# marianaGarcez/SpatialFlink

Measured on AMD Instinct MI355X. Metric: points/sec per window (kNN k=50, range r) at 1/2/4/8 MI355X; % HBM roofline, higher is better.
Workload: dtype f64

## Files before the change

### spatialflink_amd/csrc/gf_internal.hpp

```cpp
#pragma once

#include <hip/hip_runtime.h>

#include <cstdint>
#include <string>
#include <vector>

#include "../../include/geoflink_hip.h"
#include "gf_text.hpp"
#include "gf_numerics.hpp"

struct gf_ctx {
  int device = 0;
  hipStream_t stream = nullptr;
  hipStream_t own_stream = nullptr;
  std::string last_error;
  int timing = 0;
  int timing_period = 1;
  int64_t timing_seq[GF_K_COUNT] = {};
  struct Ev { hipEvent_t a, b; int kid; };
  std::vector<Ev> pending;
  std::vector<hipEvent_t> pool;
  std::vector<hipEvent_t> order_pool;
  double acc_ms[GF_K_COUNT] = {};
  int64_t acc_n[GF_K_COUNT] = {};
  void* scratch = nullptr;
  size_t scratch_bytes = 0;
  void* pinned = nullptr;
  size_t pinned_bytes = 0;
  int num_cus = 256;
  int join_legacy = 0;
  int join_coarse = 0;
  int join_stream = 0;
  int geojson_walk = 0;
  int geojson_wave = 0;
  unsigned long long* geojson_check = nullptr;
  int64_t csv_mean_line[2] = {0, 0};
  int join_async_done = 0;
  double join_ppp = 0.0;
  hipStream_t aux = nullptr;
  hipStream_t aux2 = nullptr;
  gf_objid_dict* dict = nullptr;
  unsigned long long* expand_ticket = nullptr;
  unsigned long long expand_base = 0;
  unsigned long long* expand_status = nullptr;
  int64_t expand_status_cap = 0;
  uint32_t expand_epoch = 0;
  unsigned long long* join_gctr = nullptr;
  unsigned long long* join_hint = nullptr;
  void* csv_head = nullptr;
  uint64_t* join_hist = nullptr;
  unsigned long long* join_ovf = nullptr;
  int64_t join_hint_no = 0;
};

struct gf_objid_dict {
  gf_ctx* ctx = nullptr;
  void* slots = nullptr;
  uint64_t cap = 0;
  char* arena = nullptr;
  uint64_t arena_cap = 0;
  unsigned long long* counters = nullptr;
  unsigned long long* idmap = nullptr;
  uint64_t idmap_cap = 0;
  int64_t size = 0;
  uint32_t round = 2;
  void* work[3] = {nullptr, nullptr, nullptr};
  uint64_t work_cap = 0;
  uint32_t* slot_of = nullptr;
  uint32_t* flag = nullptr;
  uint32_t* rank = nullptr;
  uint32_t* tmp = nullptr;
  uint64_t line_cap = 0;
  char* src = nullptr;
  uint64_t src_cap = 0;
  std::vector<unsigned long long> h_idmap;
  std::vector<char> h_arena;
};

namespace gf {

int set_err(gf_ctx* ctx, int code, const std::string& msg);
int hip_err(gf_ctx* ctx, hipError_t e, const char* what);
void* ctx_scratch(gf_ctx* ctx, size_t bytes, int* status);
int sync_aux(gf_ctx* ctx);
void* ctx_pinned(gf_ctx* ctx, size_t bytes, int* status);
int bind(gf_ctx* ctx);

#define GF_HIP_CHECK(ctx, call)                                   \
  do {                                                            \
    hipError_t _e = (call);                                       \
    if (_e != hipSuccess) return ::gf::hip_err((ctx), _e, #call); \
  } while (0)
// ... 36 lines not shown
struct KnnState {
  uint32_t hist[kDistBins];
  uint32_t ticket;
  uint32_t pad;
  double T;
  double s_pre;
  unsigned long long count;
  double hint_T;
  unsigned long long tr[4];
  unsigned long long maybe;
};

struct KnnScanArgs {
  const double* x;
  const double* y;
  const int64_t* objID;
  int64_t begin, end;
  double qx, qy;
  QueryRect qr;
  double T, s_pre;
  int use_state;
  int metric;
  KnnState* st;
  double* cand_d;
  uint32_t* cand_i;
  int64_t* cand_o;
  unsigned long long cap;
};

struct KnnSampleArgs {
  const double* x;
  const double* y;
  int64_t n;
  double qx, qy;
  QueryRect qr;
  double r, s_r;
  int32_t k;
  int metric;
  int use_hint;
  KnnState* st;
};

struct PolyView {
  const int32_t* ring_off;
  const int32_t* vert_off;
  const double* vx;
  const double* vy;
  const double* ring_env;
  int metric;
  const uint8_t* rect;
};

constexpr int kChainRun = 32;
constexpr int kChainPlainRuns = 2;
constexpr int kChainPlainRunsValue = 4;
struct ChainView {
  const int32_t* run_off;
  const int32_t* vert_off;
  const double* vx;
  const double* vy;
  const double* run_env;
  int metric;
};

struct KnnPolyArgs {
  const double* x;
  const double* y;
  const int64_t* objID;
  int64_t begin, end;
  QueryRect qr;
  PolyView poly;
  double bbox[4];
  int approx;
  double r;
  int32_t k;
  int use_state;
  int use_hint;
  KnnState* st;
  double* cand_d;
  uint32_t* cand_i;
  int64_t* cand_o;
  unsigned long long cap;
  uint32_t* maybe_i;
};

struct KnnSelectArgs {
  KnnState* st;
  const double* cand_d;
  const uint32_t* cand_i;
  const int64_t* cand_o;
  unsigned long long cap;
  int use_state;
  double T;
  double r;
  int32_t k;
  int write_hint;
  int64_t idx_base;
  void* result;
};

constexpr int kRangeMaxParts = 4096;
constexpr int kRangeTicketSlot = 2 * kRangeMaxParts;

struct RangeArgs {
  const double* x;
  const double* y;
  int64_t n;
  uint64_t* bitmap;
  uint64_t* multi;
  uint64_t* partials;
  int64_t* counts;
  int32_t nq;
  QueryRect qr;
  int32_t grid_n;
  double minX, minY, cl;
  const uint8_t* table;
  const uint32_t* rows;
  const uint32_t* rowoff;
  const uint8_t* spans;
  int32_t span_bytes;
  int32_t span_lds;
  const double* xt;
  const double* yt;
  double x_lo, x_hi, y_lo, y_hi;
  double sx_lo, sx_hi;
  double sy_lo, sy_hi;
  int span_mode;
  double inv_cl;
  const int32_t* extra;
  int32_t n_extra;
  const int32_t* cand_off;
  const int32_t* cand_list;
  int approx;
  int metric;
  double r, s_r;
  double thr;
  double qx0, qy0;
  const double* qx;
  const double* qy;
  int32_t npoly;
  const int32_t* ring_off;
  const int32_t* vert_off;
  const double* vx;
  const double* vy;
  const double* bbox;
  const double* ring_env;
  uint32_t* queue;
  uint32_t* queue_count;
  double* queue_xy;
  int64_t seg_cap;
  int32_t drain_lanes;
  const uint8_t* rect;
  const int32_t* brect;
  int32_t g_layers, c_layers;
};

hipError_t launch_assign(gf_ctx* ctx, const gf_grid* g, const gf_points* p, int32_t* cx, int32_t* cy);
hipError_t launch_histogram(hipStream_t s, const uint32_t* keys, int64_t n, uint32_t* hist);
constexpr int kRadixMaxBits = 9;
constexpr int kRadixMaxDigits = 1 << kRadixMaxBits;
constexpr int kRadixThreads = 1024;
constexpr int kRadixTile = 8192;
#ifndef GF_BUCKET_BITS
#define GF_BUCKET_BITS 9
#endif
constexpr int kBucketBits = GF_BUCKET_BITS;
// ... 447 lines not shown
  int64_t nt;
  uint32_t* tlist[2];
  uint32_t* tlen[2];
  const uint32_t* toff[2];
  int64_t m, npts;
  int64_t* c_keys;
  double* c_x;
  double* c_y;
  int64_t* c_ts;
  uint32_t* c_idx;
};
enum TjoinStage {
  kTjoinQueryKeys = 0,
  kTjoinQueryRank = 1,
  kTjoinQueryScatter = 2,
  kTjoinRunStarts = 3,
  kTjoinRunEnds = 4,
  kTjoinCellKeys = 5,
  kTjoinProbe = 6,
  kTjoinOccupied = 7,
  kTjoinCompact = 8,
  kTjoinRows = 9,
  kTjoinRowSlots = 10,
  kTjoinSideList = 11,
  kTjoinTotals = 12,
  kTjoinGather = 13,
};
hipError_t launch_tjoin(gf_ctx* ctx, int stage, const TjoinArgs& a);

struct TrangeArgs {
  const double* x;
  const double* y;
  int64_t n;
  const uint32_t* did;
  uint32_t* hit;
  uint64_t* bitmap;
  int32_t grid_n;
  double minX, minY, cl;
  const uint8_t* cls;
  const int32_t* cand_off;
  const int32_t* cand_list;
  const int32_t* extra;
  int32_t n_extra;
  PolyView poly;
  const uint8_t* wide;
  uint2* work;
  uint32_t work_cap;
  unsigned long long* ctr;
  int64_t* count;
};
enum TrangeStage {
  kTrangeMark = 0,
  kTrangeWaves = 1,
  kTrangeCount = 2,
};
hipError_t launch_trange(gf_ctx* ctx, int stage, const TrangeArgs& a);

hipError_t launch_knn_sample(gf_ctx* ctx, const KnnSampleArgs& a);
hipError_t launch_knn_scan(gf_ctx* ctx, const KnnScanArgs& a, int blocks, int unroll, int nt);
hipError_t launch_knn_select(gf_ctx* ctx, const KnnSelectArgs& a);
struct KnnLargeArgs {
  const double* cd;
  const int64_t* co;
  const uint32_t* ci;
  uint32_t* perm;
  int64_t m;
  int field;
  uint32_t* keys;
  uint32_t* out;
  uint32_t* cnt;
  int pass;
  unsigned long long* lane_count;
  unsigned long long* lane_maybe;
  int32_t k;
  double T;
  int64_t idx_base;
  void* result;
};
hipError_t launch_knn_large(gf_ctx* ctx, int op, const KnnLargeArgs& a);
constexpr int32_t kMaxKLarge = 1 << 24;
int knn_exact_record(gf_knn_plan* P, const gf_points* pts, void* result);

hipError_t launch_knn_poly_sample(gf_ctx* ctx, const KnnPolyArgs& a, int chain);
hipError_t launch_knn_poly_scan(gf_ctx* ctx, const KnnPolyArgs& a, int blocks, int chain);
struct KnnSelectArgs;
struct KnnMergeArgs;
hipError_t launch_knn_poly_fused(gf_ctx* ctx, const KnnPolyArgs& a, const KnnSelectArgs& prev, int has_prev,
                                 int blocks, const KnnMergeArgs* merge, int chain);
__host__ __device__ inline size_t merge_any_hash(int64_t e) {
  size_t h = 1024;
  while (h < 2 * (size_t)e) h <<= 1;
  return h;
}
__host__ __device__ inline size_t merge_any_bytes(int32_t nrec, int32_t k) {
  const int64_t e = (int64_t)nrec * k;
  return ((size_t)e * 24 + merge_any_hash(e) * 12 + 255) & ~(size_t)255;
}
hipError_t launch_knn_merge(gf_ctx* ctx, int32_t k, const void* records, int32_t nrec, size_t rec_stride,
                            int32_t nwin, size_t win_stride, void* result, size_t res_stride, int foreign,
                            void* scratch);
__host__ __device__ inline size_t str_side_off(int32_t k) { return ((size_t)4 * (k + 1) + 7) & ~(size_t)7; }
__host__ __device__ inline size_t str_record_bytes(int32_t k, int64_t cap) {
  return 32 + (size_t)24 * k + 16 + str_side_off(k) + (((size_t)cap + 7) & ~(size_t)7);
}
__host__ __device__ inline size_t strmerge_pow2(int64_t e) {
  size_t p = 2;
  while (p < (size_t)e) p <<= 1;
  return p;
}
__host__ __device__ inline size_t strmerge_bytes(int32_t nrec, int32_t k) {
  const int64_t e = (int64_t)nrec * k;
  return ((size_t)e * 40 + strmerge_pow2(e) * 4 + strmerge_pow2(2 * e) * 8 + (size_t)k * 16 + 1024) & ~(size_t)255;
}
hipError_t launch_knn_attach_strings(gf_ctx* ctx, int32_t k, const unsigned long long* idmap, const char* arena,
                                     int64_t dict_size, const void* records, int32_t nrec, int64_t cap, void* out);
hipError_t launch_knn_merge_strings(gf_ctx* ctx, int32_t k, int64_t cap, const void* records, int32_t nrec,
                                    size_t rec_stride, int32_t nwin, size_t win_stride, void* results, void* scratch);
constexpr int kMaxMergeRecs = 64;
struct KnnRecList {
  const char* rec[kMaxMergeRecs];
};
hipError_t launch_knn_merge_list(gf_ctx* ctx, int32_t k, const KnnRecList& list, int32_t nrec, void* result,
                                 void* scratch);
constexpr int kFusedMergeMaxK = 128;
struct KnnMergeArgs {
  int32_t nrec;
  void* result;
  KnnRecList list;
};
hipError_t launch_knn_fused(gf_ctx* ctx, const KnnScanArgs& a, const KnnSelectArgs& prev, int has_prev,
                            int scan_blocks, int unroll, int nt, const KnnMergeArgs* merge);
int knn_enqueue_merge(gf_knn_plan* P, const gf_points* pts, void* result, const KnnMergeArgs* merge, int* merged);
bool knn_select_pending(const gf_knn_plan* P);

hipError_t launch_range(gf_ctx* ctx, const RangeArgs& a, int table_mode, int poly, int blocks);
struct RangeWin {
  const double* x;
  const double* y;
  int64_t n;
  uint64_t* bitmap;
  uint64_t* multi;
  uint64_t* partials;
  int64_t* counts;
};
struct RangeBatch {
  RangeWin w[kRangeBatchMax];
};
hipError_t launch_range_batch(gf_ctx* ctx, const RangeArgs& a, const RangeBatch& b, int nwin, int table_mode, int poly,
                              int blocks);
struct RangeGatherArgs {
  const uint32_t* list[kMaxMergeRecs];
  const int64_t* cnt[kMaxMergeRecs];
  int64_t base[kMaxMergeRecs];
  int32_t npanes;
  int64_t total;
  uint32_t* out;
  int64_t* count;
};
hipError_t launch_range_window_gather(hipStream_t s, const RangeGatherArgs& a);
hipError_t launch_join_ppoly(gf_ctx* ctx, const RangeArgs& a, int blocks, int jblocks, uint32_t* ecnt, uint32_t* ecand,
                             uint32_t* btot, unsigned long long* total, uint32_t* pairs, int64_t cap, int aligned,
                             int poly);

struct JoinArgs {
  const double* ox;
  const double* oy;
  int64_t no;
  double u_minX, u_minY, u_cl;
  int32_t qn;
  int64_t c;
  const uint32_t* q_off;
// ... 143 lines not shown
  int64_t span_bytes = 0;
  double* xt = nullptr;
  double* yt = nullptr;
  double x_lo = 0, x_hi = 0, y_lo = 0, y_hi = 0;
  double sx_lo = 0, sx_hi = 0;
  double sy_lo = 0, sy_hi = 0;
  double span_frac = 1.0;
  int32_t* extra = nullptr;
  int32_t n_extra = 0;
  int32_t* cand_off = nullptr;
  int32_t* cand_list = nullptr;
  double* qx = nullptr;
  double* qy = nullptr;
  int32_t npoly = 0;
  int32_t* ring_off = nullptr;
  int32_t* vert_off = nullptr;
  double* vx = nullptr;
  double* vy = nullptr;
  double* bbox = nullptr;
  double* ring_env = nullptr;
  uint64_t* partials = nullptr;
  uint64_t* batch_partials = nullptr;
  int blocks = 0;
  uint32_t* queue = nullptr;
  double* queue_xy = nullptr;
  int64_t queue_cap = 0;
  uint32_t* queue_count = nullptr;
  int64_t cls_cells[4] = {0, 0, 0, 0};
  int32_t scan_blocks = 0;
  int32_t defer_mode = 0;
  int32_t drain_lanes = 0;
  int join = 0;
  int32_t* brect = nullptr;
  uint8_t* rect = nullptr;
  uint32_t* jecnt = nullptr;
  uint32_t* jecand = nullptr;
  uint32_t* jbtot = nullptr;
  unsigned long long* jtotal = nullptr;
  int chain_mode = 0;
  int32_t* run_off = nullptr;
  double* run_env = nullptr;
};

struct gf_knn_plan {
  gf_ctx* ctx = nullptr;
  gf_grid grid{};
  double qx = 0, qy = 0, r = 0;
  int32_t k = 0;
  int metric = 0;
  gf::QueryRect qr{};
  struct Lane {
    gf::KnnState* st = nullptr;
    double* cand_d = nullptr;
    uint32_t* cand_i = nullptr;
    int64_t* cand_o = nullptr;
  } lane[6];
  int64_t cap = 0;
  int pipeline = 1;
  uint64_t seq = 0;
  int lane_warm[6] = {0, 0, 0, 0, 0, 0};
  struct Pend {
    int lane;
    void* result;
    int64_t idx_base;
    uint64_t seq;
  };
  Pend pq[3];
  int npq = 0;
  int use_hint = 1;
  int64_t idx_base = 0;
  void* tmp_result = nullptr;
  void* host_result = nullptr;
  int scan_blocks = 0;
  int scan_unroll = 2;
  int scan_nt = 1;
  int large = 0;
  int poly = 0, approx = 0;
  int32_t* ring_off = nullptr;
  int32_t* vert_off = nullptr;
  double* vx = nullptr;
  double* vy = nullptr;
  double* ring_env = nullptr;
  double bbox[4] = {0, 0, 0, 0};
  uint32_t* maybe_i[3] = {nullptr, nullptr, nullptr};
  int64_t maybe_cap = 0;
  int chain_mode = 0;
};

struct gf_window {
  gf_ctx* ctx = nullptr;
  int64_t capacity = 0, n = 0;
  double* x = nullptr;
  double* y = nullptr;
  int64_t* objID = nullptr;
  int64_t* ts = nullptr;
  bool has_objid = false, has_ts = false;
  const int64_t* objid_mapped = nullptr;
  hipStream_t copy = nullptr;
  hipEvent_t ready = nullptr, fence_main = nullptr, fence_aux = nullptr, fence_aux2 = nullptr;
  bool pending = false;
};
```

### spatialflink_amd/csrc/k_knn.hip

```cpp
#define GF_TU_NAME k_knn_hip
#include "gf_buildtag.hpp"

#include <type_traits>

#include "gf_geom.hpp"
#include "gf_internal.hpp"

namespace gf {

__device__ __forceinline__ bool classify_cg(const QueryRect& q, double px, double py) {
  const double xs = (px == px) ? px : q.minX;
  const double ys = (py == py) ? py : q.minY;
  const bool inG = q.g_any && in_iv(q.gx, xs) && in_iv(q.gy, ys);
  return inG || (in_iv(q.cgx, xs) && in_iv(q.cgy, ys));
}

template <int METRIC>
__device__ __forceinline__ bool knn_pass(double qx, double qy, const QueryRect& qr, double px, double py,
                                         double sp, double T) {
  const double dx = qx - px, dy = qy - py;
  const double s = dx * dx + dy * dy;
  if (!(s <= sp)) return false;
  if (!classify_cg(qr, px, py)) return false;
  return METRIC == 0 ? true : fdlibm_hypot(dx, dy) <= T;
// ... 1072 lines not shown
                                                               void* result) {
  __shared__ SelFull L;
  const ListRecs src{&list};
  knn_merge_body(k, src, nrec, result, L);
}

hipError_t launch_knn_merge(gf_ctx* ctx, int32_t k, const void* records, int32_t nrec, size_t rec_stride,
                            int32_t nwin, size_t win_stride, void* result, size_t res_stride, int foreign,
                            void* scratch) {
  KTimer t(ctx, GF_K_KNN_MERGE);
  if (k > kMaxK)
    hipLaunchKernelGGL(knn_merge_any_kernel, dim3(nwin), dim3(kMergeAnyT), 0, ctx->stream, k, (const char*)records,
                       nrec, rec_stride, win_stride, result, res_stride, foreign, (char*)scratch,
                       merge_any_bytes(nrec, k));
  else
    hipLaunchKernelGGL(knn_merge_kernel, dim3(nwin), dim3(kSelT), 0, ctx->stream, k, (const char*)records, nrec,
                       rec_stride, win_stride, result, res_stride, foreign);
  return hipGetLastError();
}

hipError_t launch_knn_merge_list(gf_ctx* ctx, int32_t k, const KnnRecList& list, int32_t nrec, void* result,
                                 void* scratch) {
  KTimer t(ctx, GF_K_KNN_MERGE);
  if (k > kMaxK)
    hipLaunchKernelGGL(knn_merge_any_list_kernel, dim3(1), dim3(kMergeAnyT), 0, ctx->stream, k, list, nrec, result,
                       (char*)scratch);
  else
    hipLaunchKernelGGL(knn_merge_list_kernel, dim3(1), dim3(kSelT), 0, ctx->stream, k, list, nrec, result);
  return hipGetLastError();
}

template <int CHAIN>
__device__ __forceinline__ double poly_exact_distance(const KnnPolyArgs& a, double px, double py, double T) {
  if constexpr (CHAIN)
    return chain_distance<true>(px, py, ChainView{a.poly.ring_off, a.poly.vert_off, a.poly.vx, a.poly.vy, a.poly.ring_env,
                                                  a.poly.metric}, 0, T);
  else
    return polygon_distance(px, py, a.poly, 0);
}

template <int CHAIN>
__device__ __forceinline__ bool poly_pass(const KnnPolyArgs& a, double px, double py, double T, double& d) {
  if (!classify_cg(a.qr, px, py)) return false;
  if (px == px && py == py && env_far(a.bbox, px, py, T)) return false;
  d = a.approx ? point_bbox_distance(px, py, a.bbox) : poly_exact_distance<CHAIN>(a, px, py, T);
  return d <= T;
}

template <int CHAIN>
__global__ __launch_bounds__(kBlock) void knn_poly_sample_kernel(KnnPolyArgs a) {
  __shared__ uint32_t lh[kDistBins];
  if (a.use_hint) {
    const double h = a.st->hint_T;
    if (h > 0.0) {
      if (blockIdx.x == 0 && threadIdx.x == 0) a.st->T = h < a.r ? h : a.r;
      return;
    }
  }
  for (int j = threadIdx.x; j < kDistBins; j += kBlock) lh[j] = 0u;
  __syncthreads();
  const int64_t n = a.end - a.begin;
  const int64_t stride = n / gridDim.x;
  const int64_t p0 = a.begin + (int64_t)blockIdx.x * stride;
  const int64_t bbase = dist_bin_base(a.r);
  for (int u = threadIdx.x; u < kSamplePerBlock; u += kBlock) {
    const double px = a.x[p0 + u], py = a.y[p0 + u];
    double d;
    if (poly_pass<CHAIN>(a, px, py, a.r, d)) atomicAdd(&lh[dist_bin(d, bbase)], 1u);
  }
  sample_finish(a.st, lh, a.k, a.r, a.poly.metric, bbase);
}

__device__ __forceinline__ bool poly_maybe(const KnnPolyArgs& a, double px, double py, double T) {
  if (!classify_cg(a.qr, px, py)) return false;
  return !(px == px && py == py && env_far(a.bbox, px, py, T));
}

__device__ __forceinline__ void maybe_append(const KnnPolyArgs& a, bool c, int64_t i) {
  wave_reserve(&a.st->maybe, c, [&](unsigned long long pos) {
    if (pos < a.cap) a.maybe_i[pos] = (uint32_t)i;
  });
}

__device__ __forceinline__ void knn_poly_scan_body(const KnnPolyArgs& a, double T, int64_t bid, int64_t nblk) {
  const int lane = threadIdx.x & 63;
  const int64_t stride = nblk * kBlock;
  const int64_t pb = a.begin >> 1, pe = a.end >> 1;
  for (int64_t p = pb + bid * kBlock + threadIdx.x; p - lane < pe; p += stride) {
    const bool in = p < pe;
    dbl2 xv = {0.0, 0.0}, yv = {0.0, 0.0};
    if (in) {
      xv = __builtin_nontemporal_load(reinterpret_cast<const dbl2*>(a.x) + p);
      yv = __builtin_nontemporal_load(reinterpret_cast<const dbl2*>(a.y) + p);
    }
    const bool c0 = in && poly_maybe(a, xv.x, yv.x, T);
    const bool c1 = in && poly_maybe(a, xv.y, yv.y, T);
    if (__ballot(c0 || c1) == 0) continue;
    maybe_append(a, c0, 2 * p);
    maybe_append(a, c1, 2 * p + 1);
  }
  if ((a.end & 1) && bid == 0 && threadIdx.x < 64) {
    const int64_t i = a.end - 1;
    maybe_append(a, lane == 0 && poly_maybe(a, a.x[i], a.y[i], T), i);
  }
}

__global__ __launch_bounds__(kBlock) void knn_poly_scan_kernel(KnnPolyArgs a) {
  knn_poly_scan_body(a, a.use_state ? a.st->T : a.r, blockIdx.x, gridDim.x);
}

__global__ __launch_bounds__(kBlock) void knn_poly_fused_kernel(KnnPolyArgs a, KnnSelectArgs prev, int has_prev,
                                                                KnnMergeArgs m) {
  __shared__ SelLite L;
  if (blockIdx.x == 0) {
    fused_block0(prev, has_prev, m, L);
    return;
  }
  double T;
  if (a.use_state == 2) {
    T = a.st->T;
  } else {
    const double h = a.st->hint_T;
    T = (h > 0.0 && h < a.r) ? h : a.r;
    if (blockIdx.x == 1 && threadIdx.x == 0) a.st->T = T;
  }
  knn_poly_scan_body(a, T, blockIdx.x - 1, gridDim.x - 1);
}

template <int CHAIN>
__global__ __launch_bounds__(kBlock) void knn_poly_refine_kernel(KnnPolyArgs a) {
  const double T = a.use_state ? a.st->T : a.r;
  const unsigned long long nm = a.st->maybe;
  if (nm > a.cap) {
    if (blockIdx.x == 0 && threadIdx.x == 0) atomicAdd(&a.st->count, nm);
    return;
  }
  const int lane = threadIdx.x & 63;
  const int64_t stride = (int64_t)gridDim.x * kBlock;
  for (int64_t j = (int64_t)blockIdx.x * kBlock + threadIdx.x; j - lane < (int64_t)nm; j += stride) {
    const bool in = j < (int64_t)nm;
    const int64_t i = in ? (int64_t)a.maybe_i[j] : 0;
    double d = 0.0;
    bool c = false;
    if (in) {
      const double px = a.x[i], py = a.y[i];
      d = a.approx ? point_bbox_distance(px, py, a.bbox) : poly_exact_distance<CHAIN>(a, px, py, T);
      c = d <= T;
    }
    wave_reserve(&a.st->count, c, [&a, d, i](unsigned long long pos) {
      if (pos < a.cap) {
        a.cand_d[pos] = d;
        a.cand_i[pos] = (uint32_t)i;
        a.cand_o[pos] = a.objID[i];
      }
    });
  }
}

hipError_t launch_knn_poly_sample(gf_ctx* ctx, const KnnPolyArgs& a, int chain) {
  KTimer t(ctx, GF_K_KNN_SAMPLE);
  if (chain) hipLaunchKernelGGL(knn_poly_sample_kernel<1>, dim3(kSampleBlocks), dim3(kBlock), 0, ctx->stream, a);
  else hipLaunchKernelGGL(knn_poly_sample_kernel<0>, dim3(kSampleBlocks), dim3(kBlock), 0, ctx->stream, a);
  return hipGetLastError();
}

static void launch_knn_poly_refine(gf_ctx* ctx, const KnnPolyArgs& a, int chain) {
  if (chain) hipLaunchKernelGGL(knn_poly_refine_kernel<1>, dim3(256), dim3(kBlock), 0, ctx->stream, a);
  else hipLaunchKernelGGL(knn_poly_refine_kernel<0>, dim3(256), dim3(kBlock), 0, ctx->stream, a);
}

hipError_t launch_knn_poly_fused(gf_ctx* ctx, const KnnPolyArgs& a, const KnnSelectArgs& prev, int has_prev,
                                 int blocks, const KnnMergeArgs* merge, int chain) {
  KnnMergeArgs m{};
  if (merge && has_prev) m = *merge;
  {
    KTimer t(ctx, GF_K_KNN_SCAN);
    hipLaunchKernelGGL(knn_poly_fused_kernel, dim3(blocks + 1), dim3(kBlock), 0, ctx->stream, a, prev, has_prev, m);
  }
  KnnPolyArgs r = a;
  r.use_state = 1;
  launch_knn_poly_refine(ctx, r, chain);
  return hipGetLastError();
}

hipError_t launch_knn_poly_scan(gf_ctx* ctx, const KnnPolyArgs& a, int blocks, int chain) {
  {
    KTimer t(ctx, GF_K_KNN_SCAN);
    hipLaunchKernelGGL(knn_poly_scan_kernel, dim3(blocks), dim3(kBlock), 0, ctx->stream, a);
  }
  launch_knn_poly_refine(ctx, a, chain);
  return hipGetLastError();
}

struct StrSide {
  int32_t status;
  int32_t n;
  int64_t nbytes;
};
__device__ __forceinline__ StrSide* side_of(void* rec, int32_t k) {
  return reinterpret_cast<StrSide*>((char*)rec + 32 + (size_t)24 * k);
}
__device__ __forceinline__ uint32_t* side_off(void* rec, int32_t k) { return reinterpret_cast<uint32_t*>(side_of(rec, k) + 1); }
__device__ __forceinline__ char* side_bytes(void* rec, int32_t k) { return (char*)side_off(rec, k) + str_side_off(k); }
__device__ __forceinline__ bool dict_key(int64_t o) { return o < GF_OBJID_NUMERIC_MIN; }

template <int NT>
__device__ __forceinline__ uint32_t block_excl(uint32_t v, uint32_t* excl, uint32_t* ws) {
  const int lane = threadIdx.x & 63, w = threadIdx.x >> 6;
  uint32_t inc = v;
#pragma unroll
  for (int o = 1; o < 64; o <<= 1) {
    const uint32_t t = __shfl_up(inc, o, 64);
    if (lane >= o) inc += t;
  }
  if (lane == 63) ws[w] = inc;
  __syncthreads();
  uint32_t before = 0, tot = 0;
#pragma unroll
  for (int i = 0; i < NT / 64; ++i) {
    before += i < w ? ws[i] : 0u;
    tot += ws[i];
  }
  *excl = before + inc - v;
  __syncthreads();
  return tot;
}

template <int NT, class Len, class Src>
__device__ void side_pack(void* rec, int32_t k, int n, int64_t cap, const Len& len_of, const Src& src_of, uint32_t* ws) {
  StrSide* sd = side_of(rec, k);
  uint32_t* off = side_off(rec, k);
  char* bytes = side_bytes(rec, k);
  uint32_t carry = 0;
  for (int i0 = 0; i0 < n; i0 += NT) {
    const int i = i0 + (int)threadIdx.x;
    const uint32_t l = i < n ? len_of(i) : 0u;
    uint32_t ex;
    const uint32_t tot = block_excl<NT>(l, &ex, ws);
    if (i < n) off[i] = carry + ex;
    carry += tot;
  }
  const bool fits = (int64_t)carry <= cap;
  if (fits)
    for (int i = threadIdx.x; i < n; i += NT) {
      const uint32_t l = len_of(i);
      const char* src = src_of(i);
      char* dst = bytes + off[i];
      for (uint32_t b = 0; b < l; ++b) dst[b] = src[b];
    }
  if (threadIdx.x == 0) {
    off[n] = carry;
    sd->status = fits ? 0 : 1;
    sd->n = n;
    sd->nbytes = (int64_t)carry;
  }
}

__global__ __launch_bounds__(kBlock) void knn_attach_strings_kernel(int32_t k, const unsigned long long* idmap,
                                                                    const char* arena, int64_t dict_size,
                                                                    const char* records, int64_t cap, char* out) {
  __shared__ uint32_t ws[kBlock / 64];
  const size_t rb = 32 + (size_t)24 * k;
  const char* in = records + (size_t)blockIdx.x * rb;
  char* o = out + (size_t)blockIdx.x * str_record_bytes(k, cap);
  for (size_t b = (size_t)threadIdx.x * 8; b < rb; b += (size_t)kBlock * 8)
    *reinterpret_cast<uint64_t*>(o + b) = *reinterpret_cast<const uint64_t*>(in + b);
  const gf_knn_header* h = reinterpret_cast<const gf_knn_header*>(in);
  const int n = h->status == 0 ? h->n : 0;
  const RecView v = rec_view((void*)in, k);
  auto meta = [&](int i) -> unsigned long long {
    const int64_t key = v.o[i];
// ... 182 lines not shown
```

### spatialflink_amd/csrc/knn.cpp

```cpp
#define GF_TU_NAME knn_cpp
#include "gf_buildtag.hpp"

#include <hip/hip_runtime.h>

#include <initializer_list>
#include <iterator>
#include <limits>
#include <unordered_set>

#include "gf_chain_plan.hpp"
#include "gf_host.hpp"

using namespace gf;

extern "C" size_t gf_knn_result_bytes(int32_t k) {
  return sizeof(gf_knn_header) + (size_t)(k > 0 ? k : 0) * (sizeof(double) + 2 * sizeof(int64_t));
}

extern "C" void gf_knn_plan_destroy(gf_knn_plan* P) {
  if (!P) return;
  hipSetDevice(P->ctx->device);
  hipStreamSynchronize(P->ctx->stream);
  for (auto& L : P->lane) {
    if (L.st) hipFree(L.st);
// ... 11 lines not shown
}

static int knn_alloc_lane(gf_knn_plan* P, int j, int64_t cap) {
  gf_ctx* ctx = P->ctx;
  gf_knn_plan::Lane& L = P->lane[j];
  if (!L.st) {
    GF_HIP_CHECK(ctx, hipMalloc(&L.st, sizeof(KnnState)));
    GF_HIP_CHECK(ctx, hipMemset(L.st, 0, sizeof(KnnState)));
  }
  if (L.cand_d) hipFree(L.cand_d);
  if (L.cand_i) hipFree(L.cand_i);
  if (L.cand_o) hipFree(L.cand_o);
  L.cand_d = nullptr;
  L.cand_i = nullptr;
  L.cand_o = nullptr;
  GF_HIP_CHECK(ctx, hipMalloc(&L.cand_d, sizeof(double) * (size_t)cap));
  GF_HIP_CHECK(ctx, hipMalloc(&L.cand_i, sizeof(uint32_t) * (size_t)cap));
  GF_HIP_CHECK(ctx, hipMalloc(&L.cand_o, sizeof(int64_t) * (size_t)cap));
  return GF_OK;
}

static int knn_alloc_candidates(gf_knn_plan* P, int64_t cap) {
  int st;
  GF_HIP_CHECK(P->ctx, hipStreamSynchronize(P->ctx->stream));
  if (int e = sync_aux(P->ctx)) return e;
  for (int j = 0; j < (int)std::size(P->lane); ++j)
    if ((j == 0 || P->lane[j].st) && (st = knn_alloc_lane(P, j, cap))) return st;
  P->cap = cap;
  return GF_OK;
}

extern "C" int gf_knn_pp_plan_create(gf_ctx* ctx, const gf_grid* g, double qx, double qy, double r, int32_t k,
                                     int metric, gf_knn_plan** out) {
  if (!ctx || !out || !grid_ok(g) || k < 1 || k > kMaxKLarge || (metric != 0 && metric != 1))
    return set_err(ctx, GF_ERR_ARG, "gf_knn_pp_plan_create: bad argument (k must be in [1, 2^24])");
  *out = nullptr;
  int st = bind(ctx);
  if (st) return st;
  gf_knn_plan* P = new gf_knn_plan();
  P->ctx = ctx;
  P->grid = *g;
  P->qx = qx; P->qy = qy; P->r = r; P->k = k; P->metric = metric;
  const int32_t gl = guaranteed_layers(g->cellLength, r), cl = candidate_layers(g->cellLength, r);
  const int32_t qcx = cell_index(qx, g->minX, g->cellLength), qcy = cell_index(qy, g->minY, g->cellLength);
  P->qr = make_qrect(*g, qcx, qcy, gl, cl);
  auto fail = [&](int s) { gf_knn_plan_destroy(P); return s; };
  hipError_t e;
  if ((st = knn_alloc_candidates(P, (int64_t)1 << 20))) return fail(st);
  if ((e = hipMalloc(&P->tmp_result, gf_knn_result_bytes(k))) != hipSuccess) return fail(hip_err(ctx, e, "hipMalloc"));
  if ((e = hipHostMalloc(&P->host_result, gf_knn_result_bytes(k), hipHostMallocDefault)) != hipSuccess)
    return fail(hip_err(ctx, e, "hipHostMalloc"));
  P->scan_blocks = 0;
  P->large = k > kMaxK;
  *out = P;
  return GF_OK;
}

static void bbox_query_rect(gf_knn_plan* P, const gf_grid* g, double r) {
  const int32_t gl = guaranteed_layers(g->cellLength, r), cl = candidate_layers(g->cellLength, r);
  const int64_t bx0 = cell_index(P->bbox[0], g->minX, g->cellLength), bx1 = cell_index(P->bbox[2], g->minX, g->cellLength);
  const int64_t by0 = cell_index(P->bbox[1], g->minY, g->cellLength), by1 = cell_index(P->bbox[3], g->minY, g->cellLength);
  const double nan = std::numeric_limits<double>::quiet_NaN();
  const int64_t n1 = g->n - 1;
  QueryRect q;
  q.minX = g->minX;
  q.minY = g->minY;
  if (cl > 0) {
    q.cgx = axis_iv(std::max<int64_t>(bx0 - cl, 0), std::min<int64_t>(bx1 + cl, n1), g->minX, g->cellLength);
    q.cgy = axis_iv(std::max<int64_t>(by0 - cl, 0), std::min<int64_t>(by1 + cl, n1), g->minY, g->cellLength);
  } else {
    q.cgx = q.cgy = {nan, nan};
  }
  if (gl > 0) {
    q.gx = axis_iv(std::max<int64_t>(bx0 - gl, 0), std::min<int64_t>(bx1 + gl, n1), g->minX, g->cellLength);
    q.gy = axis_iv(std::max<int64_t>(by0 - gl, 0), std::min<int64_t>(by1 + gl, n1), g->minY, g->cellLength);
  } else if (gl == 0) {
    q.gx = axis_iv(bx0, bx1, g->minX, g->cellLength);
    q.gy = axis_iv(by0, by1, g->minY, g->cellLength);
  } else {
    q.gx = q.gy = {nan, nan};
  }
  q.g_any = (gl >= 0) && !std::isnan(q.gx.lo) && !std::isnan(q.gy.lo);
  P->qr = q;
}

extern "C" int gf_knn_ppoly_plan_create(gf_ctx* ctx, const gf_grid* g, const gf_polygons* poly, double r,
                                        int32_t k, int approximate, int metric, gf_knn_plan** out) {
  if (!ctx || !out || !grid_ok(g) || !poly || poly->npoly != 1 || k < 1 || k > kMaxKLarge || (metric != 0 && metric != 1))
    return set_err(ctx, GF_ERR_ARG, "gf_knn_ppoly_plan_create: bad argument (one polygon, 1 <= k <= 2^24)");
  *out = nullptr;
  const int32_t nrings = poly->ring_off[1] - poly->ring_off[0];
  if (poly->ring_off[0] != 0 || nrings < 1) return set_err(ctx, GF_ERR_ARG, "polygon without a shell");
  for (int32_t j = 0; j < nrings; ++j) {
    const int32_t v0 = poly->vert_off[j], v1 = poly->vert_off[j + 1];
    if (v1 - v0 < 4 || poly->vx[v0] != poly->vx[v1 - 1] || poly->vy[v0] != poly->vy[v1 - 1])
      return set_err(ctx, GF_ERR_ARG, "ring must be closed with >= 4 vertices");
  }
  int st = gf_knn_pp_plan_create(ctx, g, 0.0, 0.0, r, k, metric, out);
  if (st) return st;
  gf_knn_plan* P = *out;
  *out = nullptr;
  P->poly = 1;
  P->approx = approximate != 0;
  std::vector<double> renv(4 * (size_t)nrings);
  for (int32_t j = 0; j < nrings; ++j) {
    const int32_t v0 = poly->vert_off[j], v1 = poly->vert_off[j + 1];
    double mnx = poly->vx[v0], mxx = mnx, mny = poly->vy[v0], mxy = mny;
    for (int32_t v = v0 + 1; v < v1; ++v) {
      mnx = std::min(mnx, poly->vx[v]); mxx = std::max(mxx, poly->vx[v]);
      mny = std::min(mny, poly->vy[v]); mxy = std::max(mxy, poly->vy[v]);
    }
    renv[4 * j] = mnx; renv[4 * j + 1] = mxx; renv[4 * j + 2] = mny; renv[4 * j + 3] = mxy;
  }
  P->bbox[0] = renv[0]; P->bbox[1] = renv[2]; P->bbox[2] = renv[1]; P->bbox[3] = renv[3];
  bbox_query_rect(P, g, r);
  const int32_t nverts = poly->vert_off[nrings];
  std::vector<int32_t> ro = {0, nrings}, vo(poly->vert_off, poly->vert_off + nrings + 1);
  std::vector<double> vx(poly->vx, poly->vx + nverts), vy(poly->vy, poly->vy + nverts);
  if ((st = upload(ctx, &P->ring_off, ro)) || (st = upload(ctx, &P->vert_off, vo)) || (st = upload(ctx, &P->vx, vx)) ||
      (st = upload(ctx, &P->vy, vy)) || (st = upload(ctx, &P->ring_env, renv))) {
    gf_knn_plan_destroy(P);
    return st;
  }
  *out = P;
  return GF_OK;
}

extern "C" int gf_knn_pls_plan_create(gf_ctx* ctx, const gf_grid* g, const gf_linestrings* lines, double r,
                                      int32_t k, int approximate, int metric, gf_knn_plan** out) {
  if (!ctx || !out || !grid_ok(g) || !chain_valid(lines) || lines->nline != 1 || k < 1 || k > kMaxKLarge ||
      (metric != 0 && metric != 1))
    return set_err(ctx, GF_ERR_ARG, "gf_knn_pls_plan_create: bad argument (one line of >= 2 vertices, 1 <= k <= 2^24)");
  *out = nullptr;
  int st = gf_knn_pp_plan_create(ctx, g, 0.0, 0.0, r, k, metric, out);
  if (st) return st;
  gf_knn_plan* P = *out;
  *out = nullptr;
  P->poly = 2;
  P->approx = approximate != 0;
  ChainTables T;
  chain_build(*lines, kChainRun, T);
  for (int i = 0; i < 4; ++i) P->bbox[i] = T.bbox[i];
  bbox_query_rect(P, g, r);
  if ((st = upload(ctx, &P->ring_off, T.run_off)) || (st = upload(ctx, &P->vert_off, T.vert_off)) ||
      (st = upload(ctx, &P->vx, T.vx)) || (st = upload(ctx, &P->vy, T.vy)) || (st = upload(ctx, &P->ring_env, T.run_env))) {
    gf_knn_plan_destroy(P);
    return st;
  }
  *out = P;
  return GF_OK;
}

extern "C" int gf_knn_plan_set_chain_mode(gf_knn_plan* P, int mode) {
  if (!P || P->poly != 2 || (mode != 0 && mode != 1)) return GF_ERR_ARG;
  P->chain_mode = mode;
  return GF_OK;
}

extern "C" int gf_knn_plan_set_capacity(gf_knn_plan* P, int64_t cap) {
  if (!P || cap < 2 || cap > (int64_t)1 << 31) return GF_ERR_ARG;
  int st = bind(P->ctx);
  if (st) return st;
  int fs = gf_knn_plan_flush(P);
  if (fs) return fs;
  hipStreamSynchronize(P->ctx->stream);
  return knn_alloc_candidates(P, cap & ~(int64_t)1);
}

extern "C" int gf_knn_plan_set_tuning(gf_knn_plan* P, int32_t scan_blocks, int32_t unroll, int32_t nontemporal) {
  if (!P || scan_blocks < 0 || unroll < 1 || unroll > 8) return GF_ERR_ARG;
  P->scan_blocks = scan_blocks;
  P->scan_unroll = unroll;
  P->scan_nt = nontemporal != 0;
  return GF_OK;
}

extern "C" int gf_knn_plan_set_index_base(gf_knn_plan* P, int64_t base) {
  if (!P || base < 0) return GF_ERR_ARG;
  P->idx_base = base;
  return GF_OK;
}

static int knn_streams(const gf_knn_plan* P) { return P->pipeline >= 2 ? P->pipeline - 1 : 1; }

static hipStream_t knn_stream(gf_ctx* ctx, int s) { return s == 0 ? ctx->stream : (s == 1 ? ctx->aux : ctx->aux2); }

static KnnScanArgs scan_args(gf_knn_plan* P, int j, const gf_points* pts, int64_t begin, int64_t end, int use_state) {
  const gf_knn_plan::Lane& L = P->lane[j];
  KnnScanArgs s{};
  s.x = pts->x; s.y = pts->y; s.objID = pts->objID; s.begin = begin; s.end = end;
  s.qx = P->qx; s.qy = P->qy; s.qr = P->qr;
  s.T = P->r; s.s_pre = s_prefilter(P->r, P->metric);
  s.use_state = use_state; s.metric = P->metric; s.st = L.st;
  s.cand_d = L.cand_d; s.cand_i = L.cand_i; s.cand_o = L.cand_o; s.cap = (unsigned long long)P->cap;
  return s;
}

static KnnSelectArgs select_args(gf_knn_plan* P, int j, int use_state, int write_hint, void* result,
                                 int64_t idx_base) {
  const gf_knn_plan::Lane& L = P->lane[j];
  KnnSelectArgs q{};
  q.st = L.st; q.cand_d = L.cand_d; q.cand_i = L.cand_i; q.cand_o = L.cand_o;
  q.cap = (unsigned long long)P->cap;
  q.use_state = use_state; q.T = P->r; q.r = P->r; q.k = P->k; q.result = result;
  q.write_hint = write_hint; q.idx_base = idx_base;
  return q;
}

static KnnPolyArgs poly_args(gf_knn_plan* P, int j, const gf_points* pts, int64_t begin, int64_t end, int use_state,
                             int use_hint) {
  const gf_knn_plan::Lane& L = P->lane[j];
  KnnPolyArgs a{};
  a.x = pts->x; a.y = pts->y; a.objID = pts->objID; a.begin = begin; a.end = end;
  a.qr = P->qr;
  a.poly = PolyView{P->ring_off, P->vert_off, P->vx, P->vy, P->ring_env, P->metric};
  if (P->poly == 2 && P->chain_mode == 1) a.poly.ring_off = nullptr;
  for (int i = 0; i < 4; ++i) a.bbox[i] = P->bbox[i];
  a.approx = P->approx; a.r = P->r; a.k = P->k; a.use_state = use_state; a.use_hint = use_hint;
  a.st = L.st; a.cand_d = L.cand_d; a.cand_i = L.cand_i; a.cand_o = L.cand_o; a.cap = (unsigned long long)P->cap;
  a.maybe_i = P->maybe_i[j % knn_streams(P)];
  return a;
}

static int poly_buffers(gf_knn_plan* P) {
  if (P->maybe_cap >= P->cap) return GF_OK;
  GF_HIP_CHECK(P->ctx, hipStreamSynchronize(P->ctx->stream));
  if (int e = sync_aux(P->ctx)) return e;
  for (auto& m : P->maybe_i) {
    if (m) hipFree(m);
    m = nullptr;
    GF_HIP_CHECK(P->ctx, hipMalloc(&m, sizeof(uint32_t) * (size_t)P->cap));
  }
  P->maybe_cap = P->cap;
  return GF_OK;
}

static int scan_blocks_for(gf_knn_plan* P, int64_t n) {
  if (P->scan_blocks > 0) return P->scan_blocks;
  const int64_t pairs = ((P->poly ? (n + 1) / 2 : n) + 1) / 2;
  return std::min(stream_blocks(P->ctx, pairs), P->ctx->num_cus * 4);
}

static int launch_sample(gf_knn_plan* P, int j, const gf_points* pts, int use_hint) {
  if (P->poly) {
    GF_HIP_CHECK(P->ctx, launch_knn_poly_sample(P->ctx, poly_args(P, j, pts, 0, pts->n, 1, use_hint), P->poly == 2));
    return GF_OK;
  }
  KnnSampleArgs s{};
  s.x = pts->x; s.y = pts->y; s.n = pts->n; s.qx = P->qx; s.qy = P->qy; s.qr = P->qr;
  s.r = P->r; s.s_r = s_prefilter(P->r, P->metric); s.k = P->k; s.metric = P->metric; s.st = P->lane[j].st;
  s.use_hint = use_hint;
  GF_HIP_CHECK(P->ctx, launch_knn_sample(P->ctx, s));
  return GF_OK;
}

static int launch_scan(gf_knn_plan* P, int j, const gf_points* pts, int64_t begin, int64_t end, int use_state) {
  gf_ctx* ctx = P->ctx;
  const int blocks = scan_blocks_for(P, end - begin);
  if (P->poly) {
    if (int st = poly_buffers(P)) return st;
    GF_HIP_CHECK(ctx, launch_knn_poly_scan(ctx, poly_args(P, j, pts, begin, end, use_state, 0), blocks, P->poly == 2));
  } else {
    GF_HIP_CHECK(ctx, launch_knn_scan(ctx, scan_args(P, j, pts, begin, end, use_state), blocks, P->scan_unroll,
                                      P->scan_nt));
  }
  return GF_OK;
}

static int launch_fused(gf_knn_plan* P, int j, const gf_points* pts, int use_state, const KnnSelectArgs& prev,
                        int has_prev, const KnnMergeArgs* merge) {
  gf_ctx* ctx = P->ctx;
  const int blocks = scan_blocks_for(P, pts->n);
  if (P->poly) {
    if (int st = poly_buffers(P)) return st;
    GF_HIP_CHECK(ctx, launch_knn_poly_fused(ctx, poly_args(P, j, pts, 0, pts->n, use_state, 0), prev, has_prev, blocks,
                                           merge, P->poly == 2));
  } else {
    GF_HIP_CHECK(ctx, launch_knn_fused(ctx, scan_args(P, j, pts, 0, pts->n, use_state), prev, has_prev, blocks,
                                       P->scan_unroll, P->scan_nt, merge));
  }
  return GF_OK;
}

static bool fallback_resamples(const gf_knn_plan* P) { return !P->poly; }

static int knn_scan_select(gf_knn_plan* P, int j, const gf_points* pts, int64_t begin, int64_t end, int use_state,
                           int write_hint, void* result) {
  if (int st = launch_scan(P, j, pts, begin, end, use_state)) return st;
  GF_HIP_CHECK(P->ctx, launch_knn_select(P->ctx, select_args(P, j, use_state, write_hint, result, P->idx_base)));
  return GF_OK;
}

static int knn_large(gf_knn_plan* P, const gf_points* pts, void* result) {
  gf_ctx* ctx = P->ctx;
  int st;
  const int64_t n = pts->n;
  if (P->cap < n && (st = knn_alloc_candidates(P, n))) return st;
  if ((st = launch_scan(P, 0, pts, 0, n, 0))) return st;
  const gf_knn_plan::Lane& L = P->lane[0];
  const int64_t mm = std::max<int64_t>(n, 1);
  const int nb = radix_blocks(ctx, mm);
  const int64_t mat = (int64_t)256 * nb;
  Arena ar;
  uint32_t *keys[2], *perm[2], *cnt, *m, *ms;
  ar.take(keys[0], mm); ar.take(keys[1], mm);
  ar.take(perm[0], mm); ar.take(perm[1], mm);
  ar.take(cnt, 2); ar.take(m, mat); ar.take(ms, mat + 1);
  if ((st = ar.alloc(ctx))) return st;
  KnnLargeArgs a{};
  a.cd = L.cand_d; a.co = L.cand_o; a.ci = L.cand_i; a.k = P->k; a.T = P->r; a.idx_base = P->idx_base;
  a.result = result; a.m = mm; a.cnt = cnt;
  a.lane_count = &L.st->count; a.lane_maybe = &L.st->maybe;
  GF_HIP_CHECK(ctx, launch_knn_large(ctx, 5, a));
  int cur = 0;
  auto sort_by = [&](int pass, std::initializer_list<int> fields) -> int {
    for (int f : fields) {
      a.perm = perm[cur]; a.field = f; a.keys = keys[0]; a.pass = pass;
      GF_HIP_CHECK(ctx, launch_knn_large(ctx, 1, a));
      for (int p = 0; p < 4; ++p) {
        RadixArgs r{};
        r.tile = radix_tile();
        r.n = mm; r.n_dev = a.cnt + pass;
        r.kin = keys[p & 1]; r.vin = perm[cur];
        r.kout = keys[(p + 1) & 1]; r.vout = perm[cur ^ 1];
        r.shift = p * 8; r.bits = 8; r.nblk = nb; r.M = m; r.Ms = ms;
        GF_HIP_CHECK(ctx, launch_radix(ctx, 0, r, nb));
        if (int e = scan1(ctx, m, mat, ms)) return e;
        GF_HIP_CHECK(ctx, launch_radix(ctx, 1, r, nb));
        cur ^= 1;
      }
    }
    return GF_OK;
  };
  a.perm = perm[cur];
  GF_HIP_CHECK(ctx, launch_knn_large(ctx, 0, a));
  if ((st = sort_by(0, {0, 1, 2, 3, 4}))) return st;
  a.perm = perm[cur]; a.out = perm[cur ^ 1];
  GF_HIP_CHECK(ctx, launch_knn_large(ctx, 2, a));
  cur ^= 1;
  if ((st = sort_by(1, {0, 3, 4, 1, 2}))) return st;
  a.perm = perm[cur];
  GF_HIP_CHECK(ctx, launch_knn_large(ctx, 4, a));
  return GF_OK;
}

extern "C" int gf_knn_enqueue(gf_knn_plan* P, const gf_points* pts, void* result) {
  int merged = 0;
  return gf::knn_enqueue_merge(P, pts, result, nullptr, &merged);
}

int gf::knn_enqueue_merge(gf_knn_plan* P, const gf_points* pts, void* result, const KnnMergeArgs* merge,
                          int* merged) {
  *merged = 0;
  if (!P || !result) return GF_ERR_ARG;
  gf_ctx* ctx = P->ctx;
  int st = bind(ctx);
  if (st) return st;
  if ((st = check_points(ctx, pts))) return st;
  if (pts->n > 0 && !pts->objID) return set_err(ctx, GF_ERR_ARG, "kNN needs objID");
// ... 222 lines not shown
```

Before: 792.0 billion.

## Add x-band prefilter and unrolled prefetching scan for polygon kNN

The polygon kNN scan now loads x coordinates first and tests them against a conservative band around the polygon bbox widened by the current threshold, loading y only for lanes whose x falls in the band. This cuts HBM reads of y when most points lie outside the band. The scan loop is also templated on unroll and nontemporal flags with software prefetch of the next x tile, and the poly path gets fewer blocks per CU. The band margin includes a scale-based epsilon so it does not drop true candidates, though it adds extra branches and ballots.

Result: no change. 795.1 billion (median of 6 runs) (+0.4%).

```diff
diff --git a/spatialflink_amd/csrc/gf_internal.hpp b/spatialflink_amd/csrc/gf_internal.hpp
--- a/spatialflink_amd/csrc/gf_internal.hpp
+++ b/spatialflink_amd/csrc/gf_internal.hpp
@@ -9,6 +9,7 @@
 #include "../../include/geoflink_hip.h"
 #include "gf_text.hpp"
 #include "gf_numerics.hpp"
+#include "gf_knn_band.hpp"
 
 struct gf_ctx {
   int device = 0;
@@ -211,6 +212,7 @@
   int64_t* cand_o;
   unsigned long long cap;
   uint32_t* maybe_i;
+  double band_s;
 };
 
 struct KnnSelectArgs {
@@ -824,11 +826,12 @@
 int knn_exact_record(gf_knn_plan* P, const gf_points* pts, void* result);
 
 hipError_t launch_knn_poly_sample(gf_ctx* ctx, const KnnPolyArgs& a, int chain);
-hipError_t launch_knn_poly_scan(gf_ctx* ctx, const KnnPolyArgs& a, int blocks, int chain);
+hipError_t launch_knn_poly_scan(gf_ctx* ctx, const KnnPolyArgs& a, int blocks, int unroll, int nt,
+                                int chain);
 struct KnnSelectArgs;
 struct KnnMergeArgs;
 hipError_t launch_knn_poly_fused(gf_ctx* ctx, const KnnPolyArgs& a, const KnnSelectArgs& prev, int has_prev,
-                                 int blocks, const KnnMergeArgs* merge, int chain);
+                                 int blocks, int unroll, int nt, const KnnMergeArgs* merge, int chain);
 __host__ __device__ inline size_t merge_any_hash(int64_t e) {
   size_t h = 1024;
   while (h < 2 * (size_t)e) h <<= 1;
@@ -1138,6 +1141,7 @@
   double* vy = nullptr;
   double* ring_env = nullptr;
   double bbox[4] = {0, 0, 0, 0};
+  double band_s = 0;
   uint32_t* maybe_i[3] = {nullptr, nullptr, nullptr};
   int64_t maybe_cap = 0;
   int chain_mode = 0;
diff --git a/spatialflink_amd/csrc/gf_knn_band.hpp b/spatialflink_amd/csrc/gf_knn_band.hpp
--- /dev/null
+++ b/spatialflink_amd/csrc/gf_knn_band.hpp
@@ -0,0 +1,41 @@
+#pragma once
+
+#include "gf_numerics.hpp"
+
+namespace gf {
+
+struct KnnBand {
+  double lo, hi;
+};
+
+GF_HD double band_iv_abs_max(const AxisIv& iv) {
+  const double a = fabs(iv.lo), b = fabs(iv.hi_excl);
+  if (!(a < INFINITY) || !(b < INFINITY)) return INFINITY;
+  return a > b ? a : b;
+}
+
+GF_HD double knn_band_scale(const AxisIv& cgx, const AxisIv& cgy, const AxisIv& gx, const AxisIv& gy, int g_any,
+                            const double* bbox) {
+  double xm = band_iv_abs_max(cgx), ym = band_iv_abs_max(cgy);
+  if (g_any) {
+    const double gxm = band_iv_abs_max(gx), gym = band_iv_abs_max(gy);
+    xm = gxm > xm ? gxm : xm;
+    ym = gym > ym ? gym : ym;
+  }
+  const double s = xm + ym + fabs(bbox[0]) + fabs(bbox[1]) + fabs(bbox[2]) + fabs(bbox[3]);
+  return s < INFINITY ? s : INFINITY;
+}
+
+GF_HD KnnBand knn_poly_band(const double* bbox, double T, double S) {
+  const double w0 = T + T * 1e-9 + S * 1e-12;
+  double w = w0 * (1.0 + 0x1p-20);
+  if (!(w > w0)) w = INFINITY;
+  KnnBand b;
+  b.lo = bbox[0] - w;
+  b.hi = bbox[2] + w;
+  return b;
+}
+
+GF_HD bool band_skips(const KnnBand& b, double px) { return px < b.lo || px > b.hi; }
+
+}
diff --git a/spatialflink_amd/csrc/k_knn.hip b/spatialflink_amd/csrc/k_knn.hip
--- a/spatialflink_amd/csrc/k_knn.hip
+++ b/spatialflink_amd/csrc/k_knn.hip
@@ -1178,33 +1178,104 @@
   });
 }
 
+__device__ __forceinline__ uint32_t band_bits(const KnnBand& b, const dbl2& xv) {
+  return (uint32_t)!band_skips(b, xv.x) | ((uint32_t)!band_skips(b, xv.y) << 1);
+}
+
+template <int U>
+__device__ __forceinline__ void knn_poly_tile(const KnnPolyArgs& a, const dbl2 (&xv)[U], const dbl2 (&yv)[U],
+                                              uint32_t bm, int64_t p0, int64_t wstride, double T) {
+  uint32_t cm = 0;
+#pragma unroll
+  for (int u = 0; u < U; ++u) {
+    if ((bm >> (2 * u)) & 1u) cm |= (uint32_t)poly_maybe(a, xv[u].x, yv[u].x, T) << (2 * u);
+    if ((bm >> (2 * u + 1)) & 1u) cm |= (uint32_t)poly_maybe(a, xv[u].y, yv[u].y, T) << (2 * u + 1);
+  }
+  if (__ballot(cm != 0) == 0) return;
+#pragma unroll
+  for (int u = 0; u < U; ++u) {
+    const int64_t i0 = 2 * (p0 + u * wstride);
+    maybe_append(a, (cm >> (2 * u)) & 1u, i0);
+    maybe_append(a, (cm >> (2 * u + 1)) & 1u, i0 + 1);
+  }
+}
+
+template <int U, int NT>
+__device__ __forceinline__ void knn_poly_tile_x(const KnnPolyArgs& a, const KnnBand& band, const dbl2 (&xv)[U],
+                                                const dbl2* py, int64_t p0, int64_t wstride, double T) {
+  uint32_t bm = 0;
+#pragma unroll
+  for (int u = 0; u < U; ++u) bm |= band_bits(band, xv[u]) << (2 * u);
+  if (__ballot(bm != 0) == 0) return;
+  dbl2 yv[U];
+#pragma unroll
+  for (int u = 0; u < U; ++u) {
+    yv[u].x = 0.0; yv[u].y = 0.0;
+    if ((bm >> (2 * u)) & 3u) yv[u] = ld2<NT>(py + u * wstride);
+  }
+  knn_poly_tile<U>(a, xv, yv, bm, p0, wstride, T);
+}
+
+template <int U, int NT>
 __device__ __forceinline__ void knn_poly_scan_body(const KnnPolyArgs& a, double T, int64_t bid, int64_t nblk) {
+  const KnnBand band = knn_poly_band(a.bbox, T, a.band_s);
   const int lane = threadIdx.x & 63;
-  const int64_t stride = nblk * kBlock;
-  const int64_t pb = a.begin >> 1, pe = a.end >> 1;
-  for (int64_t p = pb + bid * kBlock + threadIdx.x; p - lane < pe; p += stride) {
-    const bool in = p < pe;
-    dbl2 xv = {0.0, 0.0}, yv = {0.0, 0.0};
-    if (in) {
-      xv = __builtin_nontemporal_load(reinterpret_cast<const dbl2*>(a.x) + p);
-      yv = __builtin_nontemporal_load(reinterpret_cast<const dbl2*>(a.y) + p);
-    }
-    const bool c0 = in && poly_maybe(a, xv.x, yv.x, T);
-    const bool c1 = in && poly_maybe(a, xv.y, yv.y, T);
-    if (__ballot(c0 || c1) == 0) continue;
-    maybe_append(a, c0, 2 * p);
-    maybe_append(a, c1, 2 * p + 1);
+  const int64_t wstride = nblk * kBlock;
+  const int64_t pbeg = a.begin >> 1, pe = a.end >> 1;
+  const int64_t iters = (pe - pbeg) / (U * wstride);
+  const int64_t off = bid * kBlock + threadIdx.x;
+  const dbl2* px = reinterpret_cast<const dbl2*>(a.x) + pbeg + off;
+  const dbl2* py = reinterpret_cast<const dbl2*>(a.y) + pbeg + off;
+  dbl2 xv[U];
+  if (iters > 0) {
+#pragma unroll
+    for (int u = 0; u < U; ++u) xv[u] = ld2<NT>(px + u * wstride);
+  }
+  for (int64_t it = 0; it < iters; ++it) {
+    dbl2 xn[U];
+    px += U * wstride;
+    if (it + 1 < iters) {
+#pragma unroll
+      for (int u = 0; u < U; ++u) xn[u] = ld2<NT>(px + u * wstride);
+    } else {
+#pragma unroll
+      for (int u = 0; u < U; ++u) { xn[u].x = 0.0; xn[u].y = 0.0; }
+    }
+    knn_poly_tile_x<U, NT>(a, band, xv, py, pbeg + off + it * U * wstride, wstride, T);
+    py += U * wstride;
+#pragma unroll
+    for (int u = 0; u < U; ++u) xv[u] = xn[u];
+  }
+  for (int64_t p = pbeg + iters * U * wstride + off; p - lane < pe; p += wstride) {
+    dbl2 xt[1], yt[1];
+    xt[0].x = 0.0; xt[0].y = 0.0;
+    yt[0].x = 0.0; yt[0].y = 0.0;
+    uint32_t bm = 0;
+    if (p < pe) {
+      xt[0] = *(reinterpret_cast<const dbl2*>(a.x) + p);
+      bm = band_bits(band, xt[0]);
+    }
+    if (__ballot(bm != 0) == 0) continue;
+    if (bm) yt[0] = *(reinterpret_cast<const dbl2*>(a.y) + p);
+    knn_poly_tile<1>(a, xt, yt, bm, p, wstride, T);
   }
   if ((a.end & 1) && bid == 0 && threadIdx.x < 64) {
     const int64_t i = a.end - 1;
-    maybe_append(a, lane == 0 && poly_maybe(a, a.x[i], a.y[i], T), i);
-  }
-}
-
+    bool c = false;
+    if (lane == 0) {
+      const double x1 = a.x[i];
+      if (!band_skips(band, x1)) c = poly_maybe(a, x1, a.y[i], T);
+    }
+    maybe_append(a, c, i);
+  }
+}
+
+template <int U, int NT>
 __global__ __launch_bounds__(kBlock) void knn_poly_scan_kernel(KnnPolyArgs a) {
-  knn_poly_scan_body(a, a.use_state ? a.st->T : a.r, blockIdx.x, gridDim.x);
-}
-
+  knn_poly_scan_body<U, NT>(a, a.use_state ? a.st->T : a.r, blockIdx.x, gridDim.x);
+}
+
+template <int U, int NT>
 __global__ __launch_bounds__(kBlock) void knn_poly_fused_kernel(KnnPolyArgs a, KnnSelectArgs prev, int has_prev,
                                                                 KnnMergeArgs m) {
   __shared__ SelLite L;
@@ -1220,7 +1291,7 @@
     T = (h > 0.0 && h < a.r) ? h : a.r;
     if (blockIdx.x == 1 && threadIdx.x == 0) a.st->T = T;
   }
-  knn_poly_scan_body(a, T, blockIdx.x - 1, gridDim.x - 1);
+  knn_poly_scan_body<U, NT>(a, T, blockIdx.x - 1, gridDim.x - 1);
 }
 
 template <int CHAIN>
@@ -1265,13 +1336,25 @@
   else hipLaunchKernelGGL(knn_poly_refine_kernel<0>, dim3(256), dim3(kBlock), 0, ctx->stream, a);
 }
 
+#define GF_POLY_UNROLL(K)                                                              \
+  do {                                                                                 \
+    if (nt) {                                                                          \
+      if (unroll <= 1) K(1, 1); else if (unroll == 2) K(2, 1); else K(4, 1);           \
+    } else {                                                                           \
+      if (unroll <= 1) K(1, 0); else if (unroll == 2) K(2, 0); else K(4, 0);           \
+    }                                                                                  \
+  } while (0)
+
 hipError_t launch_knn_poly_fused(gf_ctx* ctx, const KnnPolyArgs& a, const KnnSelectArgs& prev, int has_prev,
-                                 int blocks, const KnnMergeArgs* merge, int chain) {
+                                 int blocks, int unroll, int nt, const KnnMergeArgs* merge, int chain) {
   KnnMergeArgs m{};
   if (merge && has_prev) m = *merge;
   {
     KTimer t(ctx, GF_K_KNN_SCAN);
-    hipLaunchKernelGGL(knn_poly_fused_kernel, dim3(blocks + 1), dim3(kBlock), 0, ctx->stream, a, prev, has_prev, m);
+    const dim3 g(blocks + 1), b(kBlock);
+#define GF_PFUSED(U, N) hipLaunchKernelGGL((knn_poly_fused_kernel<U, N>), g, b, 0, ctx->stream, a, prev, has_prev, m)
+    GF_POLY_UNROLL(GF_PFUSED);
+#undef GF_PFUSED
   }
   KnnPolyArgs r = a;
   r.use_state = 1;
@@ -1279,10 +1362,13 @@
   return hipGetLastError();
 }
 
-hipError_t launch_knn_poly_scan(gf_ctx* ctx, const KnnPolyArgs& a, int blocks, int chain) {
+hipError_t launch_knn_poly_scan(gf_ctx* ctx, const KnnPolyArgs& a, int blocks, int unroll, int nt, int chain) {
   {
     KTimer t(ctx, GF_K_KNN_SCAN);
-    hipLaunchKernelGGL(knn_poly_scan_kernel, dim3(blocks), dim3(kBlock), 0, ctx->stream, a);
+    const dim3 g(blocks), b(kBlock);
+#define GF_PSCAN(U, N) hipLaunchKernelGGL((knn_poly_scan_kernel<U, N>), g, b, 0, ctx->stream, a)
+    GF_POLY_UNROLL(GF_PSCAN);
+#undef GF_PSCAN
   }
   launch_knn_poly_refine(ctx, a, chain);
   return hipGetLastError();
diff --git a/spatialflink_amd/csrc/knn.cpp b/spatialflink_amd/csrc/knn.cpp
--- a/spatialflink_amd/csrc/knn.cpp
+++ b/spatialflink_amd/csrc/knn.cpp
@@ -117,6 +117,7 @@
   }
   q.g_any = (gl >= 0) && !std::isnan(q.gx.lo) && !std::isnan(q.gy.lo);
   P->qr = q;
+  P->band_s = knn_band_scale(q.cgx, q.cgy, q.gx, q.gy, q.g_any, P->bbox);
 }
 
 extern "C" int gf_knn_ppoly_plan_create(gf_ctx* ctx, const gf_grid* g, const gf_polygons* poly, double r,
@@ -254,6 +255,7 @@
   a.approx = P->approx; a.r = P->r; a.k = P->k; a.use_state = use_state; a.use_hint = use_hint;
   a.st = L.st; a.cand_d = L.cand_d; a.cand_i = L.cand_i; a.cand_o = L.cand_o; a.cap = (unsigned long long)P->cap;
   a.maybe_i = P->maybe_i[j % knn_streams(P)];
+  a.band_s = P->band_s;
   return a;
 }
 
@@ -273,7 +275,7 @@
 static int scan_blocks_for(gf_knn_plan* P, int64_t n) {
   if (P->scan_blocks > 0) return P->scan_blocks;
   const int64_t pairs = ((P->poly ? (n + 1) / 2 : n) + 1) / 2;
-  return std::min(stream_blocks(P->ctx, pairs), P->ctx->num_cus * 4);
+  return std::min(stream_blocks(P->ctx, pairs), P->ctx->num_cus * (P->poly ? 2 : 4));
 }
 
 static int launch_sample(gf_knn_plan* P, int j, const gf_points* pts, int use_hint) {
@@ -294,7 +296,8 @@
   const int blocks = scan_blocks_for(P, end - begin);
   if (P->poly) {
     if (int st = poly_buffers(P)) return st;
-    GF_HIP_CHECK(ctx, launch_knn_poly_scan(ctx, poly_args(P, j, pts, begin, end, use_state, 0), blocks, P->poly == 2));
+    GF_HIP_CHECK(ctx, launch_knn_poly_scan(ctx, poly_args(P, j, pts, begin, end, use_state, 0), blocks, P->scan_unroll,
+                                           P->scan_nt, P->poly == 2));
   } else {
     GF_HIP_CHECK(ctx, launch_knn_scan(ctx, scan_args(P, j, pts, begin, end, use_state), blocks, P->scan_unroll,
                                       P->scan_nt));
@@ -309,7 +312,7 @@
   if (P->poly) {
     if (int st = poly_buffers(P)) return st;
     GF_HIP_CHECK(ctx, launch_knn_poly_fused(ctx, poly_args(P, j, pts, 0, pts->n, use_state, 0), prev, has_prev, blocks,
-                                           merge, P->poly == 2));
+                                           P->scan_unroll, P->scan_nt, merge, P->poly == 2));
   } else {
     GF_HIP_CHECK(ctx, launch_knn_fused(ctx, scan_args(P, j, pts, 0, pts->n, use_state), prev, has_prev, blocks,
                                        P->scan_unroll, P->scan_nt, merge));
```
